# ZhangT-tech/MoCA-Video

Measured on AMD Instinct MI355X. Metric: denoising UNet-steps/sec @16x320x512 fp16, higher is better.
Workload: dtype f16

## Files before the change

### include/moca_hip.h

```cpp
#ifndef MOCA_HIP_H
#define MOCA_HIP_H

#include <stdint.h>

#ifdef __cplusplus
extern "C" {
#endif

#define MOCA_OK            0
#define MOCA_E_BADARG     -1
#define MOCA_E_LAUNCH     -2
#define MOCA_E_NODEVICE   -3
#define MOCA_E_GRAPH      -4

#define MOCA_A_LINEAR   0
#define MOCA_A_CONV3X3  1
#define MOCA_A_TCONV3   2

#define MOCA_EP_GEGLU   1
#define MOCA_EP_OUT_F32 2
#define MOCA_FORCE_SMALL_TILE 4
#define MOCA_EP_COLSUM 16
#define MOCA_EP_LN     32
#define MOCA_EP_GELU    8
// ... 45 lines not shown
    const void* prefetch;
    int32_t     up_phase;
    int32_t     reserved4_;
    const void* a2;
    int32_t     lda2;
    int32_t     k1;
    int32_t     gstat_cpg;
    int32_t     gstat_coff;
    int32_t     wgroup_rows;
    int32_t     wgroup_stride;
} moca_gemm_params;

int moca_gemm_f16(const moca_gemm_params* p, void* stream);
int moca_gemm_colsum_rows(const moca_gemm_params* p);
int moca_gemm_ln_ok(const moca_gemm_params* p);
int moca_gemm_rowsum_cols(const moca_gemm_params* p);
int moca_gemm_lnfold_ok(const moca_gemm_params* p);
int moca_gemm_tattn_ok(const moca_gemm_params* p);
int moca_gemm_wgroup_ok(const moca_gemm_params* p);
int moca_gemm_cat_ok(const moca_gemm_params* p);
#define MOCA_ROUTE_SMALL64   1
#define MOCA_ROUTE_SMALL128  2
#define MOCA_ROUTE_GLDS128   3
#define MOCA_ROUTE_GLDS160   4
#define MOCA_ROUTE_G4        5
#define MOCA_ROUTE_W80       6
#define MOCA_ROUTE_W80W      7
#define MOCA_ROUTE_SQ256     8
#define MOCA_ROUTE_G4P       9
#define MOCA_ROUTE_SQP       10
#define MOCA_ROUTE_TATTN     11
#define MOCA_ROUTE_WS        12
#define MOCA_ROUTE_W80H      13
int moca_gemm_route(const moca_gemm_params* p);
int moca_gemm_splitk_groupnorm_ok(const moca_gemm_params* p, int32_t HW, int32_t frames_per_stat);
int moca_gemm_splitk_groupnorm_f16(const moca_gemm_params* p, void* y, const float* gamma, const float* beta, int32_t HW,
                                   int32_t frames_per_stat, float eps, int32_t silu, int32_t write_x, void* stream);
int64_t moca_gemm_splitk_ws_bytes(int32_t M, int32_t N, int32_t splits);

int moca_groupnorm_nhwc_f16(const void* x, void* y, const float* gamma, const float* beta,
                            int32_t F, int32_t HW, int32_t C, int32_t frames_per_stat,
                            float eps, int32_t silu, float* ws, void* stream);
int64_t moca_groupnorm_ws_bytes(int32_t F, int32_t HW, int32_t C);
#define MOCA_GN_ROUTE_STREAM    1
#define MOCA_GN_ROUTE_SLAB2     2
#define MOCA_GN_ROUTE_SLAB4     3
#define MOCA_GN_ROUTE_SLAB8     4
#define MOCA_GN_ROUTE_SLABREG1  5
#define MOCA_GN_ROUTE_SLABREG2  6
#define MOCA_GN_ROUTE_SLABREG3  7
#define MOCA_GN_ROUTE_SLABREG4  8
int moca_groupnorm_route(int32_t F, int32_t HW, int32_t C, int32_t frames_per_stat);
int moca_groupnorm_nchunk(int32_t F, int32_t HW);
int moca_groupnorm_colsum_f16(const void* x, void* y, const float* gamma, const float* beta, const float* colsum,
                              int32_t tile_rows, int32_t F, int32_t HW, int32_t C, int32_t frames_per_stat,
                              float eps, int32_t silu, float* ws, void* stream);

int moca_groupnorm_fold_weights_f16(const void* w, const float* bias, const float* gamma, const float* beta, const int64_t* gstat,
                                    void* wg, float* bg, int32_t n_sg, int32_t N, int32_t K, int32_t ldw, int64_t count, float eps,
                                    void* stream);

int moca_groupnorm_gstat_f16(const void* x, void* y, const float* gamma, const float* beta, const int64_t* gstat,
                             int32_t F, int32_t HW, int32_t C, int32_t frames_per_stat,
                             float eps, int32_t silu, void* stream);
int moca_concat_channels_gstat_f16(const void* a, const void* b, void* out, int32_t F, int32_t HW, int32_t C1, int32_t C2,
                                   int32_t frames_per_stat, int64_t* gstat, void* stream);
// ... 138 lines not shown
                       int64_t per, int64_t mask_inner, float cfg_scale, float temperature, int32_t flags, void* stream);
int moca_mask_frame_sums_f32(const float* mask, float* sums, int32_t frames, int32_t HW, void* stream);

int moca_freq_mix_3d_f32(const float* x, const float* noise, const float* lpf, float* out,
                         int32_t C, int32_t T, int32_t H, int32_t W, float* ws, void* stream);
int64_t moca_freq_mix_ws_bytes(int32_t C, int32_t T, int32_t H, int32_t W);
int moca_freq_filter_f32(float* lpf, int32_t T, int32_t H, int32_t W, int32_t type, int32_t n,
                         double d_s, double d_t, void* stream);

int moca_graph_begin(void* stream);
int moca_graph_end(void* stream, void** graph_exec_out);
int moca_graph_launch(void* graph_exec, void* stream);
int moca_graph_destroy(void* graph_exec);
int moca_stream_create(void** stream_out);
int moca_stream_destroy(void* stream);
int moca_stream_sync(void* stream);
int moca_event_create(void** ev_out);
int moca_event_record(void* ev, void* stream);
int moca_event_elapsed_ms(void* ev_start, void* ev_stop, float* ms_out);
int moca_event_destroy(void* ev);

#define MOCA_TUNE_GEMM_W80   0
#define MOCA_TUNE_GEMM_G4    1
#define MOCA_TUNE_GEMM_SQ256 2
#define MOCA_TUNE_GEMM_WIDE  3
#define MOCA_TUNE_GN_SLAB    4
#define MOCA_TUNE_GEMM_G4P   5
#define MOCA_TUNE_GEMM_MF32  6
#define MOCA_TUNE_GEMM_SQP   7
#define MOCA_TUNE_SQP_WALK   8
#define MOCA_TUNE_SLAB_F16   9
#define MOCA_TUNE_GEMM_WS    10
#define MOCA_TUNE_CONV_HALO  11
#define MOCA_TUNE_COUNT      12
int moca_set_tuning(int32_t knob, int32_t value);
int moca_debug_clock_sampler(void* buf, int32_t blocks, int32_t nsamples, const int32_t* stop, void* stream);

int moca_device_info(char* name, int32_t len, int32_t* cu_count);
const char* moca_version(void);

#ifdef __cplusplus
}
#endif
#endif
```

### moca_video_amd/csrc/common.h

```cpp
#pragma once
#include <hip/hip_runtime.h>
#include <stdint.h>
#include "../../include/moca_hip.h"

typedef _Float16 half_t;
typedef _Float16 half2v __attribute__((ext_vector_type(2)));
typedef _Float16 half4v __attribute__((ext_vector_type(4)));
typedef _Float16 half8v __attribute__((ext_vector_type(8)));
typedef float    f32x4  __attribute__((ext_vector_type(4)));
typedef float    f32x16 __attribute__((ext_vector_type(16)));

#define MOCA_WAVE 64

typedef short lds_short4v __attribute__((ext_vector_type(4)));
typedef __attribute__((address_space(3))) lds_short4v* lds_short4v_ptr;
__device__ __forceinline__ half4v lds_tr_read_b64(const char* addr) {
#if defined(__HIP_DEVICE_COMPILE__)
    const lds_short4v v = __builtin_amdgcn_ds_read_tr16_b64_v4i16((lds_short4v_ptr)addr);
    return __builtin_bit_cast(half4v, v);
#else
    return half4v{0, 0, 0, 0};
#endif
}

#define MOCA_CHECK_LAUNCH()                                  \
    do {                                                     \
        hipError_t e__ = hipGetLastError();                  \
        if (e__ != hipSuccess) return MOCA_E_LAUNCH;         \
    } while (0)

static inline hipStream_t moca_stream(void* s) { return reinterpret_cast<hipStream_t>(s); }

static inline int grid_for(int64_t total) {
    int64_t g = (total + 255) / 256;
    if (g > 4096) g = 4096;
    if (g < 1) g = 1;
    return (int)g;
}

int moca_tuning_get(int knob);

bool moca_gemm_ws_ok(const moca_gemm_params& p);
int moca_gemm_ws_launch(const moca_gemm_params& p, hipStream_t st);

__device__ __forceinline__ float moca_silu(float x) {
    return x * __builtin_amdgcn_rcpf(1.0f + __builtin_amdgcn_exp2f(x * -1.4426950408889634f));
}
typedef float f32x2 __attribute__((ext_vector_type(2)));
__device__ __forceinline__ float moca_erf(float x) {
    const float ax = fabsf(x);
    const float t = __builtin_amdgcn_rcpf(1.0f + 0.3275911f * ax);
    float y = 1.061405429f;
    y = y * t - 1.453152027f;
    y = y * t + 1.421413741f;
    y = y * t - 0.284496736f;
    y = y * t + 0.254829592f;
    y = 1.0f - y * t * __builtin_amdgcn_exp2f(ax * ax * -1.4426950408889634f);
    return copysignf(y, x);
}
__device__ __forceinline__ float moca_gelu(float x) { return 0.5f * x * (1.0f + moca_erf(x * 0.70710678118654752f)); }

__device__ __forceinline__ f32x2 moca_erf2(f32x2 x) {
    const f32x2 ax = {fabsf(x[0]), fabsf(x[1])};
    const f32x2 d = ax * 0.3275911f + 1.0f;
    const f32x2 t = {__builtin_amdgcn_rcpf(d[0]), __builtin_amdgcn_rcpf(d[1])};
    f32x2 y = t * 1.061405429f - 1.453152027f;
    y = y * t + 1.421413741f;
    y = y * t - 0.284496736f;
    y = y * t + 0.254829592f;
    const f32x2 a2 = ax * ax * -1.4426950408889634f;
    const f32x2 e = {__builtin_amdgcn_exp2f(a2[0]), __builtin_amdgcn_exp2f(a2[1])};
    y = 1.0f - y * t * e;
    return f32x2{copysignf(y[0], x[0]), copysignf(y[1], x[1])};
}
#ifdef MOCA_GELU_OLD
__device__ __forceinline__ f32x2 moca_geglu2(f32x2 v, f32x2 g) {
// ... 70 lines not shown
```

### moca_video_amd/csrc/gemm.hip

```cpp
#include "gemm_launch.h"

namespace {

template <int BN, int AMODE>
__global__ __launch_bounds__(256, 2) void gemm_f16_kernel(const moca_gemm_params p) {
    constexpr int NT = BN / 64;
    constexpr int B_SLOTS = BN / 32;
    constexpr int A_BYTES = BM * ROW_BYTES;
    constexpr int B_BYTES = BN * ROW_BYTES;

    extern __shared__ __attribute__((aligned(16))) char smem[];
    char* sA = smem;
    char* sB = smem + 2 * A_BYTES;

    const int tid = threadIdx.x, lane = tid & 63, wave = tid >> 6;
    const int wave_m = wave >> 1, wave_n = wave & 1;

    const int tiles_m = (p.M + BM - 1) / BM;
    const int tiles_n = p.N / BN;
    const int nblk = tiles_m * tiles_n * p.splits;
    int logical;
    remap_block<BN>(nblk, logical);
    const int split = logical % p.splits;
    const int tile = logical / p.splits;
// ... 390 lines not shown
            half8v r;
#pragma unroll
            for (int j = 0; j < 8; ++j) {
                float a = (float)v[i][j] * s_sc[c0 + j] + s_sh[c0 + j];
                if (silu) a = moca_silu(a);
                r[j] = (half_t)a;
            }
            *reinterpret_cast<half8v*>(y + (int64_t)mrow[i] * N + ccol[i]) = r;
        }
}

template <int BN, int AMODE>
int launch_gemm(const moca_gemm_params& p, hipStream_t st) {
    const int tiles_m = (p.M + BM - 1) / BM, tiles_n = p.N / BN;
    const int nblk = tiles_m * tiles_n * p.splits;
    constexpr int lds_pipe = 2 * (BM + BN) * ROW_BYTES;
    constexpr int lds_epi = BM * BN * 4;
    constexpr int lds = lds_pipe > lds_epi ? lds_pipe : lds_epi;
    if (!dyn_lds_once<&gemm_f16_kernel<BN, AMODE>>(lds)) return MOCA_E_LAUNCH;
    hipLaunchKernelGGL((gemm_f16_kernel<BN, AMODE>), dim3(nblk), dim3(256), lds, st, p);
    MOCA_CHECK_LAUNCH();
    return MOCA_OK;
}
int launch_gemm_small(int bn, const moca_gemm_params& p, hipStream_t st) {
    if (bn == 128) return with_gather(p, [&](auto am, auto) { return launch_gemm<128, decltype(am)::value>(p, st); });
    return with_gather(p, [&](auto am, auto) { return launch_gemm<64, decltype(am)::value>(p, st); });
}

enum Route : int {
    R_NONE = 0,
    R_SMALL64 = MOCA_ROUTE_SMALL64, R_SMALL128 = MOCA_ROUTE_SMALL128, R_GLDS128 = MOCA_ROUTE_GLDS128, R_GLDS160 = MOCA_ROUTE_GLDS160,
    R_G4 = MOCA_ROUTE_G4, R_W80 = MOCA_ROUTE_W80, R_W80W = MOCA_ROUTE_W80W, R_SQ256 = MOCA_ROUTE_SQ256, R_G4P = MOCA_ROUTE_G4P,
    R_SQP = MOCA_ROUTE_SQP, R_TATTN = MOCA_ROUTE_TATTN, R_WS = MOCA_ROUTE_WS, R_W80H = MOCA_ROUTE_W80H,
};

void normalise_splits(moca_gemm_params& p) {
    if (p.splits < 1) p.splits = 1;
    if (p.splits > (p.K + BK - 1) / BK) p.splits = (p.K + BK - 1) / BK;
    if (p.splits > 1) {
        const int nkt = (p.K + BK - 1) / BK, kts = (nkt + p.splits - 1) / p.splits;
        p.splits = (nkt + kts - 1) / kts;
    }
}

inline int64_t a_span_bytes(const moca_gemm_params& p) {
    if (p.a_mode == MOCA_A_LINEAR) return ((int64_t)p.M * p.lda + 64) * 2;
    if (p.a_mode == MOCA_A_CONV3X3) return ((int64_t)(p.M / (p.outH * p.outW)) * p.inH * p.inW * p.C + 64) * 2;
    return ((int64_t)p.M * p.C + 64) * 2;
}
inline bool buffer_addressable(const moca_gemm_params& p) {
    if (p.a2 && ((int64_t)p.M * p.lda2 + 64) * 2 >= (1ll << 31)) return false;
    return a_span_bytes(p) < (1ll << 31) && (int64_t)p.N * p.ldw * 2 < (1ll << 31);
}

bool persistent_ok(const moca_gemm_params& p, int BN, int blocks) {
    if (p.a_mode != MOCA_A_LINEAR || p.splits != 1 || p.N % BN || p.K % 64 || !buffer_addressable(p)) return false;
    if (p.flags & ~(MOCA_EP_GEGLU | MOCA_EP_LNFOLD)) return false;
    if ((p.flags & MOCA_EP_GEGLU) && (p.residual || p.rowadd)) return false;
    return ((p.M + 255) / 256) * (p.N / BN) >= blocks;
}

bool halo_ok(const moca_gemm_params& p) {
    if (p.a_mode != MOCA_A_CONV3X3 || p.stride != 1 || p.up || p.up_phase || p.nopad_lo || p.splits != 1 || p.a2 || p.wgroup_rows) return false;
    if ((p.inW != 64 && p.inW != 32) || p.inH % (320 / p.inW) || p.C % 32 || p.C > 8192) return false;
    return !(p.flags & ~(MOCA_EP_COLSUM | MOCA_EP_GSTAT | MOCA_EP_ROWSUM));
}

Route route_of(const moca_gemm_params& p) {
    if (p.flags & MOCA_EP_TATTN) return R_TATTN;
    const int ws_mode = moca_tuning_get(MOCA_TUNE_GEMM_WS);
    if (ws_mode && moca_gemm_ws_ok(p) && (ws_mode == 2 || p.residual || p.M >= (1 << 17))) return R_WS;
    if (!p.a2 && p.wgroup_rows <= 0) {
        const int sqp_mode = moca_tuning_get(MOCA_TUNE_GEMM_SQP), g4p_mode = moca_tuning_get(MOCA_TUNE_GEMM_G4P);
        if (sqp_mode && persistent_ok(p, 256, SQP_BLOCKS) && (sqp_mode == 2 || (p.flags & MOCA_EP_GEGLU))) return R_SQP;
        if (g4p_mode && persistent_ok(p, 128, G4P_BLOCKS) && (g4p_mode == 2 || (p.flags & MOCA_EP_GEGLU))) return R_G4P;
    }
    const int w80_mode = moca_tuning_get(MOCA_TUNE_GEMM_W80);
    const int tiles320 = ((p.M + 319) / 320) * (p.N / 160);
    const bool halo = moca_tuning_get(MOCA_TUNE_CONV_HALO) && halo_ok(p);
    if (w80_mode && p.N % 160 == 0 && !(p.flags & (MOCA_EP_GEGLU | MOCA_EP_OUT_F32 | MOCA_FORCE_SMALL_TILE)) && p.M > 160 &&
        (tiles320 * p.splits >= 200 || w80_mode == 2) && (fast_gather(p) || halo) && buffer_addressable(p)) {
        if (halo) return R_W80H;
        if (p.flags & MOCA_EP_LN) return R_W80W;
        const int wide_mode = moca_tuning_get(MOCA_TUNE_GEMM_WIDE);
        if (wide_mode == 0 || p.N % 320) return R_W80;
        return (p.a_mode == MOCA_A_LINEAR || wide_mode == 2) ? R_W80W : R_W80;
    }
    const int g4_mode = moca_tuning_get(MOCA_TUNE_GEMM_G4);
    const bool use_g4 = !(p.flags & MOCA_EP_OUT_F32) &&
                        (g4_mode == 2 || (g4_mode == 1 && (p.flags & MOCA_EP_GEGLU) && p.K <= 640 && p.M < (1 << 17)));
    const int sq256_mode = moca_tuning_get(MOCA_TUNE_GEMM_SQ256);
    if (sq256_mode && p.a_mode == MOCA_A_LINEAR && p.N % 256 == 0 && p.N >= 2560 && p.M >= 512 && fast_gather(p) && buffer_addressable(p) &&
        !(p.flags & (MOCA_EP_OUT_F32 | MOCA_FORCE_SMALL_TILE)) && ((p.M + 255) / 256) * (p.N / 256) * p.splits >= 200 &&
        (sq256_mode == 2 || !use_g4)) return R_SQ256;
    const int big_bn = (p.N % 128 == 0) ? 128 : (p.N % 160 == 0 ? 160 : 0);
    if (big_bn != 0 && p.M > 128 && !(p.flags & MOCA_FORCE_SMALL_TILE)) {
        if (big_bn == 128) return use_g4 ? R_G4 : R_GLDS128;
        return R_GLDS160;
    }
    return p.N % 128 == 0 ? R_SMALL128 : R_SMALL64;
}

constexpr int CAN_SPLITK = 1 << 16, CAN_A2 = 1 << 17, CAN_WGROUP = 1 << 18, CAN_UP_PHASE = 1 << 19;
constexpr int EP_STATS = MOCA_EP_COLSUM | MOCA_EP_GSTAT;
struct RouteInfo { int tm, tn, can; };
RouteInfo route_info(Route r) {
    constexpr int GLDS = MOCA_EP_GEGLU | MOCA_EP_OUT_F32 | EP_STATS | MOCA_EP_ROWSUM | MOCA_EP_LNFOLD | CAN_SPLITK | CAN_UP_PHASE;
    constexpr int W80 = EP_STATS | MOCA_EP_ROWSUM | MOCA_EP_LNFOLD | CAN_SPLITK | CAN_UP_PHASE | CAN_A2 | CAN_WGROUP;
    switch (r) {
        case R_SMALL64: return {BM, 64, MOCA_EP_OUT_F32 | MOCA_EP_GELU | CAN_SPLITK};
        case R_SMALL128: return {BM, 128, MOCA_EP_GEGLU | MOCA_EP_OUT_F32 | MOCA_EP_GELU | CAN_SPLITK};
        case R_GLDS128: return {256, 128, GLDS};
        case R_GLDS160: return {256, 160, GLDS};
        case R_G4: return {256, 128, MOCA_EP_GEGLU | MOCA_EP_LNFOLD | CAN_SPLITK | CAN_UP_PHASE};
        case R_W80: return {320, 160, W80};
        case R_W80H: return {320, 160, EP_STATS | MOCA_EP_ROWSUM};
        case R_W80W: return {160, 320, W80 | MOCA_EP_LN};
        case R_SQ256: return {256, 256, MOCA_EP_GEGLU | MOCA_EP_LNFOLD | CAN_SPLITK};
        case R_G4P: return {256, 128, MOCA_EP_GEGLU | MOCA_EP_LNFOLD};
        case R_SQP: return {256, 256, MOCA_EP_GEGLU | MOCA_EP_LNFOLD};
        case R_TATTN: return {320, 192, MOCA_EP_TATTN | MOCA_EP_LNFOLD};
        case R_WS: return {32, 80, MOCA_EP_ROWSUM | MOCA_EP_GSTAT | CAN_WGROUP};
        case R_NONE: break;
    }
    return {0, 0, 0};
}

bool route_can(Route r, const moca_gemm_params& p) {
    const RouteInfo ri = route_info(r);
    const int f = p.flags & ~(MOCA_FORCE_SMALL_TILE | MOCA_EP_SLABS);
    const int wants = f | (p.splits > 1 ? CAN_SPLITK : 0) | (p.a2 ? CAN_A2 : 0) | (p.wgroup_rows ? CAN_WGROUP : 0) | (p.up_phase ? CAN_UP_PHASE : 0);
    if (r == R_NONE || (wants & ~ri.can) || p.wgroup_rows < 0) return false;
    if (r == R_WS) return true;
    const bool linear1 = p.a_mode == MOCA_A_LINEAR && p.splits == 1;
    if (r == R_TATTN) {
        if (!linear1 || !fast_gather(p) || !buffer_addressable(p) || p.residual || p.rowadd || (p.flags & MOCA_FORCE_SMALL_TILE)) return false;
        if (p.N % 192 || p.T != 16 || p.HW <= 0 || p.HW % 20 || p.M % (16 * p.HW)) return false;
        if (p.ldo % 4 || p.ldo < p.N / 3) return false;
        return p.tattn_causal == 0 || (p.tattn_causal == 1 && p.tattn_scale > 0.f);
    }
    if ((f & EP_STATS) && (p.splits != 1 || (f & (MOCA_EP_GEGLU | MOCA_EP_OUT_F32)))) return false;
    if ((f & MOCA_EP_ROWSUM) && (p.splits != 1 || (f & (MOCA_EP_GEGLU | MOCA_EP_OUT_F32 | EP_STATS | MOCA_EP_LN | MOCA_EP_GELU)))) return false;
    if ((f & MOCA_EP_LN) && !(linear1 && p.N == 320 && !(f & EP_STATS))) return false;
    if ((f & MOCA_EP_LNFOLD) && !(linear1 && !(f & (MOCA_EP_OUT_F32 | EP_STATS | MOCA_EP_LN | MOCA_EP_ROWSUM | MOCA_EP_GELU)) &&
                                  !((r == R_GLDS128 || r == R_GLDS160) && (f & MOCA_EP_GEGLU)))) return false;
    if ((f & MOCA_EP_GELU) && (f & MOCA_EP_GEGLU)) return false;
    if (p.a2) {
        if (!linear1 || (f & ~(EP_STATS | MOCA_EP_ROWSUM))) return false;
        if (p.k1 <= 0 || p.k1 >= p.K || p.k1 % 64 || (p.K - p.k1) % 64 || p.lda % 8 || p.lda2 % 8 || p.lda < p.k1 || p.lda2 < p.K - p.k1) return false;
    }
    if (p.wgroup_rows) {
        if (!linear1 || p.a2 || p.wgroup_stride < p.N * p.ldw || (f & ~(EP_STATS | MOCA_EP_ROWSUM | MOCA_EP_LN))) return false;
        if (p.M % p.wgroup_rows || p.wgroup_rows % ri.tm) return false;
        if ((int64_t)(p.M / p.wgroup_rows) * p.wgroup_stride * 2 >= (1ll << 31)) return false;
    }
    if (p.up_phase && (p.splits != 1 || p.M <= 160 || !fast_gather(p) || p.residual || p.rowadd || (f & ~MOCA_EP_GSTAT) ||
                       (p.N % 128 && p.N % 160))) return false;
    return true;
}

Route checked_route(const moca_gemm_params& p) {
    const Route r = route_of(p);
    return route_can(r, p) ? r : R_NONE;
}

Route query_route(const moca_gemm_params* pp, int flag, moca_gemm_params& p) {
// ... 44 lines not shown
            if (p.up && (p.stride != 1 || p.outH != 2 * p.inH || p.outW != 2 * p.inW)) return R_NONE;
            if (!p.up && p.stride == 1 && (p.outH != p.inH || p.outW != p.inW)) return R_NONE;
            if (p.stride == 2 && (p.outH != (p.inH - 1) / 2 + 1 || p.outW != (p.inW - 1) / 2 + 1)) return R_NONE;
            if (p.M % (p.outH * p.outW)) return R_NONE;
            break;
        case MOCA_A_TCONV3:
            if (p.C % 8 || p.K != 3 * p.C || p.T <= 0 || p.HW <= 0 || p.M % (p.T * p.HW)) return R_NONE;
            break;
        default:
            return R_NONE;
    }
    if (p.a2 && p.a_mode != MOCA_A_LINEAR) return R_NONE;
    if (p.gstat_cpg < 0 || p.gstat_coff < 0 || ((p.gstat_cpg || p.gstat_coff) && !(p.flags & MOCA_EP_GSTAT))) return R_NONE;
    if (p.tattn_causal && !(p.flags & MOCA_EP_TATTN)) return R_NONE;
    const Route r = checked_route(p);
    if (r == R_NONE) return R_NONE;
    if ((p.flags & MOCA_EP_COLSUM) && !p.colsum) return R_NONE;
    if ((p.flags & MOCA_EP_LN) && !(p.ln_gamma && p.ln_beta && p.ln_out && p.ld_ln % 8 == 0)) return R_NONE;
    if ((p.flags & MOCA_EP_ROWSUM) && !p.rowsum) return R_NONE;
    if ((p.flags & MOCA_EP_LNFOLD) && !(p.lnf_part && p.lnf_wsum && p.lnf_nparts >= 1)) return R_NONE;
    if ((p.flags & MOCA_EP_GSTAT) &&
        !(p.gstat && !(p.flags & MOCA_EP_COLSUM) && p.gstat_rows > 0 && p.gstat_rows % route_info(r).tm == 0 && p.M % p.gstat_rows == 0 &&
          (p.gstat_cpg > 0 ? (p.gstat_coff + p.N - 1) / p.gstat_cpg < 32 : (p.N % 32 == 0 && p.gstat_coff == 0)))) return R_NONE;
    p.reserved4_ = 0;
    if ((int64_t)p.M * (geglu ? p.N / 2 : p.N) * 2 >= (128ll << 20)) p.reserved4_ |= 1;
    if (slab_f16(r, p)) p.reserved4_ |= 4;
    return r;
}

int launch_route(Route r, const moca_gemm_params& p, hipStream_t st) {
    switch (r) {
        case R_TATTN: return moca_gemm_w80s_launch(3, p, st);
        case R_WS: return moca_gemm_ws_launch(p, st);
        case R_SQP: return moca_gemm_sqp_launch(p, st);
        case R_G4P: return moca_gemm_g4p_launch(p, st);
        case R_W80: return moca_gemm_w80s_launch(0, p, st);
        case R_W80W: return moca_gemm_w80s_launch(1, p, st);
        case R_W80H: return moca_gemm_w80h_launch(p, st);
        case R_SQ256: return moca_gemm_w80s_launch(2, p, st);
        case R_G4: return moca_gemm_g4_launch(p, st);
        case R_GLDS128: return moca_gemm_glds_launch(128, p, st);
        case R_GLDS160: return moca_gemm_glds_launch(160, p, st);
        case R_SMALL128: return launch_gemm_small(128, p, st);
        case R_SMALL64: return launch_gemm_small(64, p, st);
        case R_NONE: break;
    }
    return MOCA_E_BADARG;
}

}

#ifdef MOCA_STAMPS
extern "C" int moca_debug_stamps(unsigned long long* host_out, int n_blocks) {
    if (n_blocks > STAMP_BLOCKS) n_blocks = STAMP_BLOCKS;
    return hipMemcpyFromSymbol(host_out, HIP_SYMBOL(g_stamps), (size_t)n_blocks * STAMP_SLOTS * 8) == hipSuccess ? 0 : -2;
}
#endif

extern "C" int moca_gemm_route(const moca_gemm_params* pp) {
    moca_gemm_params p;
    return prepare(pp, p);
}

extern "C" int moca_gemm_colsum_rows(const moca_gemm_params* pp) {
    moca_gemm_params p;
    return route_info(query_route(pp, (pp && (pp->flags & MOCA_EP_GSTAT)) ? 0 : MOCA_EP_COLSUM, p)).tm;
// ... 83 lines not shown
```

### moca_video_amd/csrc/runtime.hip

```cpp
#include "common.h"
#include <string.h>
#include <stdio.h>
#include <stdlib.h>

extern "C" int moca_graph_begin(void* stream) {
    if (hipStreamBeginCapture(moca_stream(stream), hipStreamCaptureModeThreadLocal) != hipSuccess) return MOCA_E_GRAPH;
    return MOCA_OK;
}

extern "C" int moca_graph_end(void* stream, void** graph_exec_out) {
    if (!graph_exec_out) return MOCA_E_BADARG;
    hipGraph_t g = nullptr;
    if (hipStreamEndCapture(moca_stream(stream), &g) != hipSuccess || !g) return MOCA_E_GRAPH;
    hipGraphExec_t ge = nullptr;
    hipError_t e = hipGraphInstantiate(&ge, g, nullptr, nullptr, 0);
    (void)hipGraphDestroy(g);
    if (e != hipSuccess || !ge) return MOCA_E_GRAPH;
    *graph_exec_out = reinterpret_cast<void*>(ge);
    return MOCA_OK;
}

extern "C" int moca_graph_launch(void* graph_exec, void* stream) {
    if (!graph_exec) return MOCA_E_BADARG;
    if (hipGraphLaunch(reinterpret_cast<hipGraphExec_t>(graph_exec), moca_stream(stream)) != hipSuccess) return MOCA_E_GRAPH;
// ... 65 lines not shown
    const int64_t n16 = bytes / 16;
    int blocks = (int)((n16 + 255) / 256);
    if (blocks < 1) blocks = 1;
    if (blocks > 1024) blocks = 1024;
    hipLaunchKernelGGL(zero_kernel, dim3(blocks), dim3(256), 0, moca_stream(stream), reinterpret_cast<uint4*>(ptr), n16,
                       reinterpret_cast<unsigned char*>(ptr) + n16 * 16, (int)(bytes - n16 * 16));
    MOCA_CHECK_LAUNCH();
    return MOCA_OK;
}

__global__ __launch_bounds__(64) void clock_sampler_kernel(unsigned long long* __restrict__ buf, int nsamples, const volatile int* stop) {
#if defined(__HIP_DEVICE_COMPILE__)
    if (threadIdx.x) return;
    unsigned long long* b = buf + (size_t)blockIdx.x * nsamples * 2;
    for (int i = 0; i < nsamples; ++i) {
        unsigned long long t, r;
        asm volatile("s_memtime %0\n\ts_memrealtime %1\n\ts_waitcnt lgkmcnt(0)" : "=s"(t), "=s"(r)::"memory");
        b[2 * i] = t;
        b[2 * i + 1] = r;
        if (stop && *stop) break;
        __builtin_amdgcn_s_sleep(127);
        __builtin_amdgcn_s_sleep(127);
    }
#endif
}
extern "C" int moca_debug_clock_sampler(void* buf, int32_t blocks, int32_t nsamples, const int32_t* stop, void* stream) {
    if (!buf || blocks < 1 || blocks > 64 || nsamples < 1 || nsamples > (1 << 20)) return MOCA_E_BADARG;
    hipLaunchKernelGGL(clock_sampler_kernel, dim3(blocks), dim3(64), 0, moca_stream(stream), reinterpret_cast<unsigned long long*>(buf), nsamples,
                       reinterpret_cast<const volatile int*>(stop));
    MOCA_CHECK_LAUNCH();
    return MOCA_OK;
}

static int g_tuning[MOCA_TUNE_COUNT] = {1, 1, 1, 1, 1, 1, 0, 1, 0, 0, 1, 1};
int moca_tuning_get(int knob) { return (knob >= 0 && knob < MOCA_TUNE_COUNT) ? g_tuning[knob] : 0; }
extern "C" int moca_set_tuning(int32_t knob, int32_t value) {
    if (knob < 0 || knob >= MOCA_TUNE_COUNT || value < 0 || value > 2) return MOCA_E_BADARG;
    const int old = g_tuning[knob];
    g_tuning[knob] = value;
    return old;
}
```

### moca_video_amd/lib.py

```python
from __future__ import annotations

import ctypes as C
import os

import torch

_HERE = os.path.dirname(os.path.abspath(__file__))
LIB_PATH = os.environ.get("MOCA_HIP_LIB") or os.path.join(_HERE, "libmoca_hip.so")

MOCA_A_LINEAR, MOCA_A_CONV3X3, MOCA_A_TCONV3 = 0, 1, 2
MOCA_EP_GEGLU, MOCA_EP_OUT_F32, MOCA_FORCE_SMALL_TILE, MOCA_EP_GELU, MOCA_EP_COLSUM, MOCA_EP_LN = 1, 2, 4, 8, 16, 32
MOCA_EP_ROWSUM, MOCA_EP_LNFOLD, MOCA_EP_GSTAT, MOCA_EP_TATTN, MOCA_EP_SLABS = 64, 128, 256, 512, 1024
MOCA_TUNE_GEMM_W80, MOCA_TUNE_GEMM_G4, MOCA_TUNE_GEMM_SQ256, MOCA_TUNE_GEMM_WIDE, MOCA_TUNE_GN_SLAB, MOCA_TUNE_GEMM_G4P, MOCA_TUNE_GEMM_MF32, MOCA_TUNE_GEMM_SQP, MOCA_TUNE_SQP_WALK = 0, 1, 2, 3, 4, 5, 6, 7, 8
MOCA_TUNE_SLAB_F16 = 9
MOCA_TUNE_GEMM_WS = 10
MOCA_TUNE_CONV_HALO = 11
MOCA_DDPM_X0, MOCA_DDPM_CLIP, MOCA_DDPM_SCALE, MOCA_DDPM_MASK_C0 = 1, 2, 4, 8
MOCA_BASE_SCALE, MOCA_BASE_MULTISTEP = 1, 2
(MOCA_ROUTE_SMALL64, MOCA_ROUTE_SMALL128, MOCA_ROUTE_GLDS128, MOCA_ROUTE_GLDS160, MOCA_ROUTE_G4, MOCA_ROUTE_W80, MOCA_ROUTE_W80W,
 MOCA_ROUTE_SQ256, MOCA_ROUTE_G4P, MOCA_ROUTE_SQP, MOCA_ROUTE_TATTN, MOCA_ROUTE_WS, MOCA_ROUTE_W80H) = range(1, 14)
(MOCA_GN_ROUTE_STREAM, MOCA_GN_ROUTE_SLAB2, MOCA_GN_ROUTE_SLAB4, MOCA_GN_ROUTE_SLAB8, MOCA_GN_ROUTE_SLABREG1, MOCA_GN_ROUTE_SLABREG2,
 MOCA_GN_ROUTE_SLABREG3, MOCA_GN_ROUTE_SLABREG4) = range(1, 9)

_ERR = {0: "ok", -1: "bad argument (shape/alignment contract)", -2: "HIP launch/runtime error",
        -3: "no gfx950 device", -4: "graph capture/replay failed"}


class MocaHipError(RuntimeError):
    pass


class GemmParams(C.Structure):
    _fields_ = [
        ("a", C.c_void_p), ("w", C.c_void_p), ("out", C.c_void_p), ("bias", C.c_void_p),
        ("rowadd", C.c_void_p), ("residual", C.c_void_p), ("splitk_ws", C.c_void_p),
        ("M", C.c_int32), ("N", C.c_int32), ("K", C.c_int32),
        ("lda", C.c_int32), ("ldw", C.c_int32), ("ldo", C.c_int32), ("ldr", C.c_int32), ("ld_rowadd", C.c_int32),
        ("rowadd_div", C.c_int32), ("a_mode", C.c_int32), ("C", C.c_int32),
        ("inH", C.c_int32), ("inW", C.c_int32), ("outH", C.c_int32), ("outW", C.c_int32),
        ("stride", C.c_int32), ("up", C.c_int32), ("T", C.c_int32), ("HW", C.c_int32),
        ("flags", C.c_int32), ("splits", C.c_int32), ("nopad_lo", C.c_int32), ("prefetch_kib", C.c_int32),
        ("tattn_causal", C.c_int32),
        ("colsum", C.c_void_p), ("ln_gamma", C.c_void_p), ("ln_beta", C.c_void_p), ("ln_out", C.c_void_p),
        ("ld_ln", C.c_int32), ("ln_eps", C.c_float),
        ("rowsum", C.c_void_p), ("lnf_part", C.c_void_p), ("lnf_wsum", C.c_void_p),
        ("lnf_nparts", C.c_int32), ("reserved2_", C.c_int32),
        ("gstat", C.c_void_p), ("gstat_rows", C.c_int32), ("tattn_scale", C.c_float),
        ("prefetch", C.c_void_p), ("up_phase", C.c_int32), ("reserved4_", C.c_int32),
        ("a2", C.c_void_p), ("lda2", C.c_int32), ("k1", C.c_int32), ("gstat_cpg", C.c_int32), ("gstat_coff", C.c_int32),
        ("wgroup_rows", C.c_int32), ("wgroup_stride", C.c_int32),
    ]


# ... 157 lines not shown
```

### moca_video_amd/ops.py

```python
from __future__ import annotations

import ctypes as C
import os
import torch

from . import lib as _l

_stream = None


def set_stream(handle):
    global _stream
    _stream = handle


def current_stream():
    if _stream is None:
        return torch.cuda.current_stream().cuda_stream
    return _stream


def _st():
    return C.c_void_p(current_stream())

# ... 93 lines not shown
def finish_lnfold(pw: PackedWeight) -> PackedWeight:
    pw.wsum = pw.w.float().sum(dim=1).contiguous()
    return pw


def _gemm_params(a, pw: PackedWeight, out, *, M, lda=None, mode=_l.MOCA_A_LINEAR, rowadd=None, rowadd_div=1,
                 residual=None, conv=None, tconv=None, out_f32=False, splits=1, splitk_ws=None, gelu=False, colsum=None, ln=None,
                 force_small=False, rowsum=None, lnfold=None, gstat=None, tattn=None, up_phase=0, prefetch=None, a2=None, slabs=False,
                 wgroup=None):
    p = _l.GemmParams()
    if wgroup is not None:
        p.wgroup_rows, p.wgroup_stride = wgroup
    p.up_phase = up_phase
    if a2 is not None:
        p.a2, p.lda2, p.k1 = a2[0].data_ptr(), a2[0].stride(-2), a2[1]
    if prefetch is not None:
        p.prefetch, p.prefetch_kib = prefetch.data_ptr(), (prefetch.numel() * prefetch.element_size()) >> 10
    p.a, p.w, p.out = a.data_ptr(), pw.w.data_ptr(), (out.data_ptr() if out is not None else None)
    p.bias = pw.bias.data_ptr() if pw.bias is not None else None
    p.rowadd = rowadd.data_ptr() if rowadd is not None else None
    p.residual = residual.data_ptr() if residual is not None else None
    p.splitk_ws = splitk_ws.data_ptr() if splitk_ws is not None else None
    p.M, p.N, p.K = M, pw.N, pw.K
    p.lda = lda if lda is not None else (a.stride(-2) if a.dim() >= 2 else pw.K)
    p.ldw = pw.w.stride(0)
    p.ldo = out.stride(-2) if out is not None else pw.N
    p.ldr = residual.stride(-2) if residual is not None else 0
    p.ld_rowadd = rowadd.stride(-2) if rowadd is not None else 0
    p.rowadd_div = rowadd_div
    p.a_mode = mode
    if conv is not None:
        p.C, p.inH, p.inW, p.outH, p.outW, p.stride, p.up = conv[:7]
        p.nopad_lo = conv[7] if len(conv) > 7 else 0
    if tconv is not None:
        p.C, p.T, p.HW = tconv
    p.flags = (_l.MOCA_EP_GEGLU if pw.geglu else 0) | (_l.MOCA_EP_OUT_F32 if out_f32 else 0) | \
              ((_l.MOCA_EP_GELU | _l.MOCA_FORCE_SMALL_TILE) if gelu else 0) | (_l.MOCA_EP_COLSUM if colsum is not None else 0) | \
              (_l.MOCA_FORCE_SMALL_TILE if force_small else 0)
    p.colsum = colsum.data_ptr() if colsum is not None else None
    if ln is not None:
        p.flags |= _l.MOCA_EP_LN
        p.ln_gamma, p.ln_beta = ln[0].data_ptr(), ln[1].data_ptr()
        p.ln_out = ln[2].data_ptr() if ln[2] is not None else None
        p.ld_ln = ln[2].stride(-2) if ln[2] is not None else pw.N
        p.ln_eps = ln[3]
    if rowsum is not None:
        p.flags |= _l.MOCA_EP_ROWSUM
        p.rowsum = rowsum.data_ptr() if torch.is_tensor(rowsum) else None
    if tattn is not None:
        p.flags |= _l.MOCA_EP_TATTN
        p.T, p.HW, p.tattn_scale = tattn[:3]
        p.tattn_causal = 1 if len(tattn) > 3 and tattn[3] else 0
    if gstat is not None:
        p.flags |= _l.MOCA_EP_GSTAT
        p.gstat = gstat[0].data_ptr()
        p.gstat_rows = gstat[1]
        if len(gstat) > 2:
            p.gstat_cpg, p.gstat_coff = gstat[2], gstat[3]
    if lnfold is not None:
        p.flags |= _l.MOCA_EP_LNFOLD
        p.lnf_part = lnfold[0].data_ptr() if lnfold[0] is not None else None
        p.lnf_nparts = lnfold[1]
        p.ln_eps = lnfold[2]
        p.lnf_wsum = pw.wsum.data_ptr() if pw.wsum is not None else None
    if slabs:
        p.flags |= _l.MOCA_EP_SLABS
# ... 281 lines not shown
```

Before: 63.89.

## Add narrow conv3x3 GEMM kernel for output-head convolution with few real channels

Adds a dedicated 3x3 convolution kernel for the output head, where N is padded to 64 but only a few (≤16) output channels are real. It computes only the valid channels with one 16-wide MFMA tile, stages a halo tile and the weights in LDS with register double-buffering, and writes zeros to the padded output columns. Row-band and column-tile sizes are chosen so the blocks balance across the CUs. The route is enabled by default through a new tuning knob, and it relies on pw.n_out being passed through reserved2_.

```diff
diff --git a/include/moca_hip.h b/include/moca_hip.h
--- a/include/moca_hip.h
+++ b/include/moca_hip.h
@@ -101,6 +101,7 @@
 #define MOCA_ROUTE_TATTN     11
 #define MOCA_ROUTE_WS        12
 #define MOCA_ROUTE_W80H      13
+#define MOCA_ROUTE_NARROW    14
 int moca_gemm_route(const moca_gemm_params* p);
 int moca_gemm_splitk_groupnorm_ok(const moca_gemm_params* p, int32_t HW, int32_t frames_per_stat);
 int moca_gemm_splitk_groupnorm_f16(const moca_gemm_params* p, void* y, const float* gamma, const float* beta, int32_t HW,
@@ -305,7 +306,9 @@
 #define MOCA_TUNE_SLAB_F16   9
 #define MOCA_TUNE_GEMM_WS    10
 #define MOCA_TUNE_CONV_HALO  11
-#define MOCA_TUNE_COUNT      12
+#define MOCA_TUNE_RESERVED12 12
+#define MOCA_TUNE_OUT_HEAD   13
+#define MOCA_TUNE_COUNT      14
 int moca_set_tuning(int32_t knob, int32_t value);
 int moca_debug_clock_sampler(void* buf, int32_t blocks, int32_t nsamples, const int32_t* stop, void* stream);
 
diff --git a/moca_video_amd/csrc/common.h b/moca_video_amd/csrc/common.h
--- a/moca_video_amd/csrc/common.h
+++ b/moca_video_amd/csrc/common.h
@@ -42,6 +42,8 @@
 
 bool moca_gemm_ws_ok(const moca_gemm_params& p);
 int moca_gemm_ws_launch(const moca_gemm_params& p, hipStream_t st);
+bool moca_gemm_narrow_ok(const moca_gemm_params& p);
+int moca_gemm_narrow_launch(const moca_gemm_params& p, hipStream_t st);
 
 __device__ __forceinline__ float moca_silu(float x) {
     return x * __builtin_amdgcn_rcpf(1.0f + __builtin_amdgcn_exp2f(x * -1.4426950408889634f));
diff --git a/moca_video_amd/csrc/gemm.hip b/moca_video_amd/csrc/gemm.hip
--- a/moca_video_amd/csrc/gemm.hip
+++ b/moca_video_amd/csrc/gemm.hip
@@ -446,6 +446,7 @@
     R_SMALL64 = MOCA_ROUTE_SMALL64, R_SMALL128 = MOCA_ROUTE_SMALL128, R_GLDS128 = MOCA_ROUTE_GLDS128, R_GLDS160 = MOCA_ROUTE_GLDS160,
     R_G4 = MOCA_ROUTE_G4, R_W80 = MOCA_ROUTE_W80, R_W80W = MOCA_ROUTE_W80W, R_SQ256 = MOCA_ROUTE_SQ256, R_G4P = MOCA_ROUTE_G4P,
     R_SQP = MOCA_ROUTE_SQP, R_TATTN = MOCA_ROUTE_TATTN, R_WS = MOCA_ROUTE_WS, R_W80H = MOCA_ROUTE_W80H,
+    R_NARROW = MOCA_ROUTE_NARROW,
 };
 
 void normalise_splits(moca_gemm_params& p) {
@@ -482,6 +483,7 @@
 
 Route route_of(const moca_gemm_params& p) {
     if (p.flags & MOCA_EP_TATTN) return R_TATTN;
+    if (moca_tuning_get(MOCA_TUNE_OUT_HEAD) && moca_gemm_narrow_ok(p)) return R_NARROW;
     const int ws_mode = moca_tuning_get(MOCA_TUNE_GEMM_WS);
     if (ws_mode && moca_gemm_ws_ok(p) && (ws_mode == 2 || p.residual || p.M >= (1 << 17))) return R_WS;
     if (!p.a2 && p.wgroup_rows <= 0) {
@@ -535,6 +537,7 @@
         case R_SQP: return {256, 256, MOCA_EP_GEGLU | MOCA_EP_LNFOLD};
         case R_TATTN: return {320, 192, MOCA_EP_TATTN | MOCA_EP_LNFOLD};
         case R_WS: return {32, 80, MOCA_EP_ROWSUM | MOCA_EP_GSTAT | CAN_WGROUP};
+        case R_NARROW: return {16, 64, 0};
         case R_NONE: break;
     }
     return {0, 0, 0};
@@ -545,7 +548,7 @@
     const int f = p.flags & ~(MOCA_FORCE_SMALL_TILE | MOCA_EP_SLABS);
     const int wants = f | (p.splits > 1 ? CAN_SPLITK : 0) | (p.a2 ? CAN_A2 : 0) | (p.wgroup_rows ? CAN_WGROUP : 0) | (p.up_phase ? CAN_UP_PHASE : 0);
     if (r == R_NONE || (wants & ~ri.can) || p.wgroup_rows < 0) return false;
-    if (r == R_WS) return true;
+    if (r == R_WS || r == R_NARROW) return true;
     const bool linear1 = p.a_mode == MOCA_A_LINEAR && p.splits == 1;
     if (r == R_TATTN) {
         if (!linear1 || !fast_gather(p) || !buffer_addressable(p) || p.residual || p.rowadd || (p.flags & MOCA_FORCE_SMALL_TILE)) return false;
@@ -656,6 +659,7 @@
     switch (r) {
         case R_TATTN: return moca_gemm_w80s_launch(3, p, st);
         case R_WS: return moca_gemm_ws_launch(p, st);
+        case R_NARROW: return moca_gemm_narrow_launch(p, st);
         case R_SQP: return moca_gemm_sqp_launch(p, st);
         case R_G4P: return moca_gemm_g4p_launch(p, st);
         case R_W80: return moca_gemm_w80s_launch(0, p, st);
diff --git a/moca_video_amd/csrc/gemm_narrow.hip b/moca_video_amd/csrc/gemm_narrow.hip
--- /dev/null
+++ b/moca_video_amd/csrc/gemm_narrow.hip
@@ -0,0 +1,199 @@
+#include "common.h"
+
+namespace {
+
+constexpr int NR_THREADS = 512;
+[[maybe_unused]] constexpr int NR_TPW = 3;
+constexpr int NR_MAXN = 16;
+constexpr int NR_N = 64;
+constexpr int NR_TILES = (NR_THREADS / 64) * NR_TPW;
+constexpr int NR_CUS = 256;
+
+inline void narrow_tiling(int64_t F, int H, int W, int& R, int& WT) {
+    const int nb = W / 16;
+    int d = 1;
+    for (int k = 2; k <= 4; ++k)
+        if (nb % k == 0) d = k;
+    WT = 16 * d;
+    int rmax = NR_TILES / d;
+    if (rmax > H) rmax = H;
+    int64_t best = -1;
+    R = 1;
+    for (int r = rmax; r >= 1; --r) {
+        const int64_t blocks = F * ((H + r - 1) / r) * (nb / d);
+        const int64_t cost = ((blocks + NR_CUS - 1) / NR_CUS) * (r + 2);
+        if (best < 0 || cost < best) { best = cost; R = r; }
+    }
+}
+
+template <int CS, int WT>
+__global__ __launch_bounds__(NR_THREADS, 1) void gemm_narrow_kernel(const moca_gemm_params p, const int R, const int nbands, const int ncolt) {
+#if defined(__HIP_DEVICE_COMPILE__)
+    constexpr int CH = CS / 8;
+    constexpr int PS = CS + 16;
+    constexpr int LW = WT + 2;
+    constexpr int NPIX = (NR_TILES * 16 / WT + 2) * LW;
+    constexpr int NXU = (NPIX * CH + NR_THREADS - 1) / NR_THREADS;
+    constexpr int NWU = (9 * NR_MAXN * CH + NR_THREADS - 1) / NR_THREADS;
+    static_assert(NR_THREADS % CH == 0 && ((2 * LW + 2) * PS + CS) * 2 < 65536, "a thread keeps one chunk column; ds_read immediates");
+
+    extern __shared__ __attribute__((aligned(16))) char smem[];
+
+    const int tid = threadIdx.x, lane = tid & 63, wave = tid >> 6;
+    const int H = p.inH, W = p.inW, C = p.C, nv = p.reserved2_;
+    half_t* xs = reinterpret_cast<half_t*>(smem);
+    half_t* ws = xs + (R + 2) * LW * PS;
+
+    int blk = blockIdx.x;
+    const int ct = blk % ncolt;
+    blk /= ncolt;
+    const int band = blk % nbands, f = blk / nbands;
+    const int y0 = band * R, x0 = ct * WT;
+    const half_t* xf = reinterpret_cast<const half_t*>(p.a) + (int64_t)f * H * W * C;
+    const half_t* wp = reinterpret_cast<const half_t*>(p.w);
+
+    const int c8 = tid % CH;
+    const int npix = (R + 2) * LW;
+    int goff[NXU], loff[NXU];
+#pragma unroll
+    for (int u = 0; u < NXU; ++u) {
+        const int pix = (tid + u * NR_THREADS) / CH;
+        const int i = pix / LW, j = pix - i * LW;
+        const int y = y0 - 1 + i, x = x0 - 1 + j;
+        loff[u] = pix < npix ? pix * PS + c8 * 8 : -1;
+        goff[u] = (pix < npix && y >= 0 && y < H && x >= 0 && x < W) ? (y * W + x) * C + c8 * 8 : -1;
+    }
+    const int nwch = 9 * nv * CH;
+    int gwoff[NWU], lwoff[NWU];
+#pragma unroll
+    for (int u = 0; u < NWU; ++u) {
+        const int e = tid + u * NR_THREADS;
+        const int r = e / CH, t = r / nv, n = r - t * nv;
+        gwoff[u] = e < nwch ? n * p.ldw + t * C + c8 * 8 : -1;
+        lwoff[u] = (t * NR_MAXN + n) * PS + c8 * 8;
+    }
+
+    struct stage_regs {
+        half8v xr[NXU], wr[NWU];
+    };
+    stage_regs st[2];
+    const half8v zero8 = {0, 0, 0, 0, 0, 0, 0, 0};
+    auto fetch = [&](stage_regs& r, int s) {
+        const int c0 = s * CS;
+#pragma unroll
+        for (int u = 0; u < NXU; ++u)
+            if (goff[u] >= 0) r.xr[u] = *reinterpret_cast<const half8v*>(xf + goff[u] + c0);
+#pragma unroll
+        for (int u = 0; u < NWU; ++u)
+            if (gwoff[u] >= 0) r.wr[u] = *reinterpret_cast<const half8v*>(wp + gwoff[u] + c0);
+    };
+    fetch(st[0], 0);
+
+    const int fr = lane & 15, fg = lane >> 4;
+    constexpr int tpr = WT / 16;
+    const int ntiles = R * tpr;
+    int a_off[NR_TPW];
+#pragma unroll
+    for (int q = 0; q < NR_TPW; ++q) {
+        const int tile = wave + (NR_THREADS / 64) * q;
+        const int ty = tile / tpr, seg = tile - ty * tpr;
+        a_off[q] = tile < ntiles ? (ty * LW + seg * 16 + fr) * PS + fg * 8 : -1;
+    }
+    f32x4 acc[NR_TPW];
+#pragma unroll
+    for (int q = 0; q < NR_TPW; ++q) acc[q] = f32x4{0.f, 0.f, 0.f, 0.f};
+
+    const int nslices = C / CS;
+    auto slice = [&](stage_regs& r, stage_regs& nxt, int s) {
+        if (s + 1 < nslices) fetch(nxt, s + 1);
+#pragma unroll
+        for (int u = 0; u < NXU; ++u) {
+            if (loff[u] < 0) continue;
+            *reinterpret_cast<half8v*>(xs + loff[u]) = goff[u] >= 0 ? r.xr[u] : zero8;
+        }
+#pragma unroll
+        for (int u = 0; u < NWU; ++u)
+            if (gwoff[u] >= 0) *reinterpret_cast<half8v*>(ws + lwoff[u]) = r.wr[u];
+        __syncthreads();
+#pragma unroll
+        for (int t = 0; t < 9; ++t) {
+            const int ky = t / 3, kx = t % 3;
+#pragma unroll
+            for (int ks = 0; ks < CS / 32; ++ks) {
+                half8v b = zero8;
+                if (fr < nv) b = *reinterpret_cast<const half8v*>(ws + (t * NR_MAXN + fr) * PS + ks * 32 + fg * 8);
+#pragma unroll
+                for (int q = 0; q < NR_TPW; ++q) {
+                    if (a_off[q] < 0) continue;
+                    const half8v a = *reinterpret_cast<const half8v*>(xs + a_off[q] + (ky * LW + kx) * PS + ks * 32);
+                    acc[q] = __builtin_amdgcn_mfma_f32_16x16x32_f16(b, a, acc[q], 0, 0, 0);
+                }
+            }
+        }
+        __syncthreads();
+    };
+    for (int s = 0; s < nslices; s += 2) {
+        slice(st[0], st[1], s);
+        if (s + 1 < nslices) slice(st[1], st[0], s + 1);
+    }
+
+    f32x4 bias = {0.f, 0.f, 0.f, 0.f};
+    if (p.bias) bias = *reinterpret_cast<const f32x4*>(p.bias + 4 * fg);
+    half_t* out = reinterpret_cast<half_t*>(p.out);
+#pragma unroll
+    for (int q = 0; q < NR_TPW; ++q) {
+        const int tile = wave + (NR_THREADS / 64) * q;
+        const int ty = tile / tpr, seg = tile - ty * tpr;
+        const int y = y0 + ty;
+        if (tile >= ntiles || y >= H) continue;
+        half_t* row = out + ((int64_t)f * H * W + (int64_t)y * W + x0 + seg * 16 + fr) * p.ldo;
+        half4v h;
+#pragma unroll
+        for (int i = 0; i < 4; ++i) h[i] = (half_t)(acc[q][i] + bias[i]);
+        *reinterpret_cast<half4v*>(row + 4 * fg) = h;
+        *reinterpret_cast<half8v*>(row + 16 + 8 * fg) = zero8;
+        if (fg < 2) *reinterpret_cast<half8v*>(row + 48 + 8 * fg) = zero8;
+    }
+#endif
+}
+
+template <int CS, int WT>
+int narrow_launch(const moca_gemm_params& p, int R, hipStream_t st) {
+    const int nbands = (p.inH + R - 1) / R, ncolt = p.inW / WT;
+    const int F = p.M / (p.inH * p.inW);
+    const int lds = ((R + 2) * (WT + 2) + 9 * NR_MAXN) * (CS + 16) * 2;
+    static int lds_set = 0;
+    if (lds > lds_set) {
+        if (hipFuncSetAttribute(reinterpret_cast<const void*>(&gemm_narrow_kernel<CS, WT>), hipFuncAttributeMaxDynamicSharedMemorySize, lds) != hipSuccess)
+            return MOCA_E_LAUNCH;
+        lds_set = lds;
+    }
+    hipLaunchKernelGGL((gemm_narrow_kernel<CS, WT>), dim3((unsigned)(F * nbands * ncolt)), dim3(NR_THREADS), lds, st, p, R, nbands, ncolt);
+    MOCA_CHECK_LAUNCH();
+    return MOCA_OK;
+}
+
+}
+
+bool moca_gemm_narrow_ok(const moca_gemm_params& p) {
+    if (p.a_mode != MOCA_A_CONV3X3 || p.stride != 1 || p.up || p.up_phase || p.nopad_lo || p.splits != 1 || p.flags) return false;
+    if (p.residual || p.rowadd || p.a2 || p.wgroup_rows) return false;
+    if (p.N != NR_N || p.reserved2_ < 1 || p.reserved2_ > NR_MAXN || p.ldo < NR_N || p.ldo % 8) return false;
+    if (p.inH <= 0 || p.inW <= 0 || p.inW % 16 || p.C <= 0 || p.C % 32 || p.K != 9 * p.C || p.ldw < 9 * p.C || p.ldw % 8) return false;
+    if ((int64_t)p.inH * p.inW * p.C > 0x7fffffffll || p.M % (p.inH * p.inW)) return false;
+    if ((reinterpret_cast<uintptr_t>(p.a) | reinterpret_cast<uintptr_t>(p.w) | reinterpret_cast<uintptr_t>(p.out) | reinterpret_cast<uintptr_t>(p.bias)) & 15)
+        return false;
+    return true;
+}
+
+int moca_gemm_narrow_launch(const moca_gemm_params& p, hipStream_t st) {
+    int R, WT;
+    narrow_tiling(p.M / (p.inH * p.inW), p.inH, p.inW, R, WT);
+    const bool c64 = p.C % 64 == 0;
+    switch (WT) {
+    case 16: return c64 ? narrow_launch<64, 16>(p, R, st) : narrow_launch<32, 16>(p, R, st);
+    case 32: return c64 ? narrow_launch<64, 32>(p, R, st) : narrow_launch<32, 32>(p, R, st);
+    case 48: return c64 ? narrow_launch<64, 48>(p, R, st) : narrow_launch<32, 48>(p, R, st);
+    default: return c64 ? narrow_launch<64, 64>(p, R, st) : narrow_launch<32, 64>(p, R, st);
+    }
+}
diff --git a/moca_video_amd/csrc/runtime.hip b/moca_video_amd/csrc/runtime.hip
--- a/moca_video_amd/csrc/runtime.hip
+++ b/moca_video_amd/csrc/runtime.hip
@@ -121,7 +121,7 @@
     return MOCA_OK;
 }
 
-static int g_tuning[MOCA_TUNE_COUNT] = {1, 1, 1, 1, 1, 1, 0, 1, 0, 0, 1, 1};
+static int g_tuning[MOCA_TUNE_COUNT] = {1, 1, 1, 1, 1, 1, 0, 1, 0, 0, 1, 1, 1, 1};
 int moca_tuning_get(int knob) { return (knob >= 0 && knob < MOCA_TUNE_COUNT) ? g_tuning[knob] : 0; }
 extern "C" int moca_set_tuning(int32_t knob, int32_t value) {
     if (knob < 0 || knob >= MOCA_TUNE_COUNT || value < 0 || value > 2) return MOCA_E_BADARG;
diff --git a/moca_video_amd/lib.py b/moca_video_amd/lib.py
--- a/moca_video_amd/lib.py
+++ b/moca_video_amd/lib.py
@@ -15,10 +15,11 @@
 MOCA_TUNE_SLAB_F16 = 9
 MOCA_TUNE_GEMM_WS = 10
 MOCA_TUNE_CONV_HALO = 11
+MOCA_TUNE_OUT_HEAD = 13
 MOCA_DDPM_X0, MOCA_DDPM_CLIP, MOCA_DDPM_SCALE, MOCA_DDPM_MASK_C0 = 1, 2, 4, 8
 MOCA_BASE_SCALE, MOCA_BASE_MULTISTEP = 1, 2
 (MOCA_ROUTE_SMALL64, MOCA_ROUTE_SMALL128, MOCA_ROUTE_GLDS128, MOCA_ROUTE_GLDS160, MOCA_ROUTE_G4, MOCA_ROUTE_W80, MOCA_ROUTE_W80W,
- MOCA_ROUTE_SQ256, MOCA_ROUTE_G4P, MOCA_ROUTE_SQP, MOCA_ROUTE_TATTN, MOCA_ROUTE_WS, MOCA_ROUTE_W80H) = range(1, 14)
+ MOCA_ROUTE_SQ256, MOCA_ROUTE_G4P, MOCA_ROUTE_SQP, MOCA_ROUTE_TATTN, MOCA_ROUTE_WS, MOCA_ROUTE_W80H, MOCA_ROUTE_NARROW) = range(1, 15)
 (MOCA_GN_ROUTE_STREAM, MOCA_GN_ROUTE_SLAB2, MOCA_GN_ROUTE_SLAB4, MOCA_GN_ROUTE_SLAB8, MOCA_GN_ROUTE_SLABREG1, MOCA_GN_ROUTE_SLABREG2,
  MOCA_GN_ROUTE_SLABREG3, MOCA_GN_ROUTE_SLABREG4) = range(1, 9)
 
diff --git a/moca_video_amd/ops.py b/moca_video_amd/ops.py
--- a/moca_video_amd/ops.py
+++ b/moca_video_amd/ops.py
@@ -149,6 +149,7 @@
     if conv is not None:
         p.C, p.inH, p.inW, p.outH, p.outW, p.stride, p.up = conv[:7]
         p.nopad_lo = conv[7] if len(conv) > 7 else 0
+        p.reserved2_ = pw.n_out if not pw.geglu and 0 < pw.n_out < pw.N else 0
     if tconv is not None:
         p.C, p.T, p.HW = tconv
     p.flags = (_l.MOCA_EP_GEGLU if pw.geglu else 0) | (_l.MOCA_EP_OUT_F32 if out_f32 else 0) | \
```

Result: no change. 64.04 (median of 6 runs) (+0.2%).
